# PacificBiosciences/ccs

Hardware: AMD Instinct MI355X
Metric: ZMWs/sec (HiFi reads/sec), 10-pass x 10 kb synthetic (higher is better)
Workload: dtype f32

## Files before the change

ccs_amd/csrc/ccsx_kernels.hip:

```cpp
#include <hip/hip_runtime.h>
#include <stdint.h>
#include <cstdio>
#include <cstdlib>

#include "ccsx.h"
#include "ccsx_kernels.h"
#include "wave_ops.h"

#define LANDED(x) asm volatile("" : "+v"(x))

#if (defined(CCSX_EXP_NO_FILL) || defined(CCSX_EXP_NO_SCORE) || defined(CCSX_EXP_ONE_ROUND) || defined(CCSX_EXP_ALL_VALID) || defined(CCSX_EXP_CHEAP_VALIDITY) || \
     defined(CCSX_EXP_NO_ROWS) || defined(CCSX_EXP_NO_SCORE_LOG) || defined(CCSX_EXP_SKIP_ROUND2_SCORE) || defined(CCSX_EXP_NO_QV_EXP) || defined(CCSX_EXP_REPEAT) || defined(CCSX_EXP_NO_BANDMASK) || \
     defined(CCSX_EXP_HOT_PROLOGUE) || defined(CCSX_EXIT_AFTER_PROLOGUE)) && !defined(CCSX_EXPERIMENT)
#error "CCSX_EXP_* / CCSX_EXIT_AFTER_PROLOGUE switches produce wrong results: build them with -DCCSX_EXPERIMENT (never ship such a library)"
#endif
#define CCSX_STR2(x) #x
#define CCSX_STR(x) CCSX_STR2(x)
int ccsx_kernel_is_experiment()
{
#ifdef CCSX_EXPERIMENT
    return 1;
#else
    return 0;
#endif
// ... 1656 lines not shown
                if (cf > NEGV / 2 && cf > bF) { bF = cf; kF = k; }
                if (cr > NEGV / 2 && cr > bR) { bR = cr; kR = k; }
            }
            const int wF = rfl(wave_max_i32(bF)), wR = rfl(wave_max_i32(bR));
            if (wF <= NEGV / 2 || wR <= NEGV / 2) continue;
            const int k1 = rfl(wave_min_i32(bF == wF ? kF : (1 << 30))), kr = rfl(wave_min_i32(bR == wR ? kR : (1 << 30)));
            const int k2 = nneed - 1 - kr;
            const int s1 = need_col(wb, nw, Ld, k1), s2r = Ld - need_col(wb, nw, Ld, k2);
            if (!(k1 < k2 && s1 > 0 && s2r > 0 && wF >= s1 && wR >= s2r && brF[k1] + brR[kr] <= I)) continue;
            if (lane == 0) {
                int32_t *ent = P.ent + P.ent_off[r];
                uint32_t *dm = P.dmask + P.ent_off[r];
                const int2 *OMF = (const int2 *)OsF, *OMR = (const int2 *)OsR;
                int e = ebF[k1];
                ent[k1] = e;
                for (int kq = k1; kq >= 2; --kq) { e = OMF[(size_t)kq * 64 + (e - loF[kq])].x; ent[kq - 1] = e; }
                ent[0] = 0;
                int er = ebR[kr];
                ent[k2] = I - er;
                for (int kq = kr; kq >= 1; --kq) {
                    er = (kq >= 2) ? OMR[(size_t)kq * 64 + (er - loR[kq])].x : 0;
                    ent[nneed - kq] = I - er;
                }
                for (int kq = k1 + 1; kq < k2; ++kq) ent[kq] = -(1 << 20) - 64 * kq;
                dm[0] = 0u;
                for (int kq = 1; kq < nneed; ++kq) dm[kq] = 0x7fffffffu;
                P.avalid[r] = 1; P.ascore[r] = wF + wR;
            }
            continue;
        }
        if (lane == 0) {
            int32_t *ent = P.ent + P.ent_off[r];
            uint32_t *dm = P.dmask + P.ent_off[r];
            const int2 *OMF = (const int2 *)OsF, *OMR = (const int2 *)OsR;
            int e = ks ? ebF[ks] : 0;
            ent[ks] = e;
            for (int k2 = ks; k2 >= 2; --k2) { e = OMF[(size_t)k2 * 64 + (e - loF[k2])].x; ent[k2 - 1] = e; }
            ent[0] = 0;
            const int ksr = nneed - 1 - ks;
            int er = ksr ? ebR[ksr] : 0;
            for (int kq = ksr; kq >= 1; --kq) {
                er = (kq >= 2) ? OMR[(size_t)kq * 64 + (er - loR[kq])].x : 0;
                ent[nneed - kq] = I - er;
            }
            dm[0] = 0u;
            for (int k2 = 1; k2 < nneed; ++k2) dm[k2] = 0x7fffffffu;
            P.avalid[r] = 1; P.ascore[r] = wbest;
        }
      }
    }
}

__global__ void k_post(KParams P, int pass)
{
    int z = blockIdx.x * blockDim.x + threadIdx.x;
    if (z >= P.n_zmw) return;
    const int zr = P.zref[z];
    if (pass && !(zr & ZREF_PASSBIT(pass))) return;
    const bool may_retry = !P.opts.no_fallback_draft && pass < 2;
    const int retry = pass == 0 ? ZREF_RETRY : ((zr & 255) | ZREF_RETRY2);
    if (P.zstat[z] != CCSX_SUCCESS) {
        P.np[z] = 0; P.out_fn[z] = 0; P.out_rn[z] = 0;
        if (may_retry && P.zstat[z] == CCSX_DRAFT_FAILURE) P.zref[z] = retry;
        return;
    }
    int r0 = P.read_off[z], nr = P.nfull[z], np = 0, rn = 0;
    const int f0 = P.flags[r0 + (zr & 255)];
    for (int r = 0; r < nr; ++r) {
        const int v = P.avalid[r0 + r];
        np += v;
        if (v && ((P.flags[r0 + r] ^ f0) & 1)) ++rn;
    }
    P.np[z] = np; P.out_fn[z] = np - rn; P.out_rn[z] = rn;
    if (2 * np <= nr) {
        if (may_retry) P.zref[z] = retry;
        else { P.zstat[z] = CCSX_TOO_MANY_UNUSABLE; P.nwin[z] = 0; }
    }
}

__global__ __launch_bounds__(1024) void k_wmap(KParams P)
{
    __shared__ int sTot[16], sCarry;
    const int tid = threadIdx.x, lane = tid & 63, wv = tid >> 6;
    if (tid == 0) sCarry = 0;
    __syncthreads();
    for (int z0 = 0; z0 < P.n_zmw; z0 += 1024) {
        const int z = z0 + tid;
        const int v = z < P.n_zmw ? P.nwin[z] : 0;
        const int incl = wave_scan_add_i32(v);
        if (lane == 63) sTot[wv] = incl;
        __syncthreads();
        int base = sCarry;
        for (int q = 0; q < wv; ++q) base += sTot[q];
        if (z < P.n_zmw) P.wstart[z] = base + incl - v;
        __syncthreads();
        if (tid == 1023) sCarry = base + incl;
        __syncthreads();
    }
    if (tid == 0) P.wstart[P.n_zmw] = sCarry;
}
__global__ __launch_bounds__(256) void k_wmap_fill(KParams P)
{
    const int z = blockIdx.x * 4 + (threadIdx.x >> 6), lane = threadIdx.x & 63;
    if (z >= P.n_zmw) return;
    const int a = P.wstart[z], nw = P.nwin[z];
    for (int w = lane; w < nw; w += LANES) P.wslot_zmw[a + w] = z;
}

#ifndef PW_THREADS
#define PW_THREADS 256
#endif
#ifndef PW_MINWAVES
#define PW_MINWAVES 4
#endif
#define PW_WAVES (PW_THREADS / 64)
#ifndef PW_CHUNK_READS
#define PW_CHUNK_READS 8
#endif
#ifndef PW_MAXREADS
#define PW_MAXREADS 32
#endif
#ifndef PW_LDS_BYTES
#define PW_LDS_BYTES 40960
#endif
#ifndef CTXS
#define CTXS 17
#endif
#define FILL16_MAXBW 24
#define TC_LO 56
#define TC_HI 38
#define TC_ROW 32
#define TC_STRAND ((CCSX_NOBS + 1) * TC_ROW)
#define DLC_S (33 + TC_LO)
#define DLC_TOTAL (TC_LO + DLC_S + 33 + TC_HI)
#define TAB_TAIL (2 * TC_HI - 48)
#define OBS_TC(o) ((o) * (TC_ROW * 8))
#define OBS_CODE(o) ((o) * (CTXS * 8))

struct LaneMut {
    int c, q, kA, kB, isdel, fin;
    int qoff;
    float dlA, dlL;
};

__device__ __forceinline__ LaneMut lane_mut(int type, int c, int x, const uint8_t *t, int J, int lf, const float *sDL)
{
    LaneMut L;
    const int tm1 = t[c > 0 ? c - 1 : 0];
    const int nidx = (type == 2) ? c : c + 1;
    const int tn = t[nidx < 31 ? nidx : 31];
    const int fin = (type == 2) ? (c == J) : (c + 1 == J);
    const int nx = fin ? 0 : tn;
    int pA = (c > 0) ? tm1 : lf;
    const int xA = (type == 1) ? nx : x;
    if (pA > 3) pA = (xA + 2) & 3;
    const int kA = pA * 4 + xA, kB = (type == 1) ? kA : xA * 4 + nx;
    const int q = (type == 2) ? c + 1 : c + 2;
    L.c = c; L.q = q > J ? J : q; L.isdel = (type == 1); L.fin = fin; L.qoff = (type == 2) ? 0 : 1;
    L.dlA = sDL[kA]; L.dlL = sDL[kB];
    L.kA = (type == 1 && fin) ? (CTXS - 1) : kA;
    L.kB = fin ? (CTXS - 1) : kB;
    return L;
}

typedef const float __attribute__((address_space(3))) *lds_cf;
typedef const char __attribute__((address_space(3))) *lds_cc;

typedef const uint8_t __attribute__((address_space(3))) *lds_cu8;
struct ScoreChain {
    float ap, bp, acc, b, bq;
    float2 pA, pB;
    lds_cf g, be;
    lds_cu8 op;
    int dg;
};

__device__ __forceinline__ float lanes_or_zero(unsigned long long m, float v)
{
    float r;
    asm("v_cndmask_b32_e64 %0, 0, %1, %2" : "=v"(r) : "v"(v), "s"(m));
    return r;
}

__device__ __forceinline__ void score_step(ScoreChain &s, const LaneMut &L, lds_cc tA, lds_cc tB, int pitch, unsigned lim)
{
    typedef const unsigned long long __attribute__((address_space(3))) *lds_cu64;
#ifndef CCSX_EXP_NO_BANDMASK
    const unsigned long long on = __builtin_amdgcn_uicmp((unsigned)s.dg, lim, 37 );
    const float gmm = lanes_or_zero(on, *s.g);
    const float bqn = lanes_or_zero(on, *s.be);
#else
    const float gmm = *s.g, bqn = *s.be;
#endif
    const int o256 = __mul24((int)*s.op, CTXS * 8);
    const unsigned long long va = *(lds_cu64)(tA + o256), vb = *(lds_cu64)(tB + o256);
    const float2 nA = make_float2(__uint_as_float((unsigned)va), __uint_as_float((unsigned)(va >> 32)));
    const float2 nB = make_float2(__uint_as_float((unsigned)vb), __uint_as_float((unsigned)(vb >> 32)));
    s.g += pitch; s.be += pitch; s.op += 1; s.dg -= 1;
    const float insA = s.pA.y, meA = s.pA.x, insB = s.pB.y;
    const float a = __builtin_fmaf(s.ap, insA, gmm);
    float b;
    if (L.isdel) b = a;
    else b = __builtin_fmaf(s.bp, insB, __builtin_fmaf(a, L.dlA, s.ap * meA));
    s.acc = __builtin_fmaf(b, __builtin_fmaf(L.dlL, s.bq, nB.x * bqn), s.acc);
    s.ap = a; s.bp = b; s.b = b; s.pA = nA; s.pB = nB; s.bq = bqn;
}

__device__ __forceinline__ int band_row0(int c, int I, int J2, float invJ2, int J, int Wr, int nrows)
{
    const int num = __mul24(2 * c, I) + J;
    int q = (int)((float)num * invJ2);
    const int r = num - __mul24(q, J2);
    q += (r >= J2 ? 1 : 0) - (r < 0 ? 1 : 0);
    int i0 = q - Wr;
    i0 = i0 < 0 ? 0 : i0;
    const int hi = I + 1 - nrows;
    return i0 > hi ? hi : i0;
}

__device__ __forceinline__ int dq_fix(float d)
{
    if (d < -DQ_CLAMP) d = -DQ_CLAMP;
    if (d > DQ_CLAMP) d = DQ_CLAMP;
    return (int)floorf(d * DQ_SCALE + 0.5f);
}

__device__ __forceinline__ float skip_perr(int g, float floor_)
{
    if (g < 0) g = 0;
    if (g > 12) g = 12;
    const float p = 8.0f * det_exp2f(-3.0f * (float)g);
    return p < floor_ ? floor_ : p;
}

__device__ __forceinline__ int tract_len(unsigned long long m, int x, int p, int nvis)
{
    const int lo = x - p < 0 ? 0 : x - p;
    const unsigned long long cand = m & ((2ull << x) - 1ull) & ~((1ull << lo) - 1ull);
    if (!cand) return 0;
    int best = 0;
#pragma unroll
    for (int which = 0; which < 2; ++which) {
        const int k = which ? 63 - __clzll((long long)cand) : __ffsll((long long)cand) - 1;
        const unsigned long long zb = ~m & ((1ull << k) - 1ull);
        const int i = zb ? 64 - __clzll((long long)zb) : 0;
        const int j = k + (__ffsll((long long)(~m >> k)) - 1);
        const int L = j - i + p, op = ((i == 0) || (j + p >= nvis)) ? 256 : 0;
        if (L > (best & 255)) best = L | op; else if (L == (best & 255)) best |= op;
    }
    return best;
}


struct FillBand { int dlo, dhi, bw, pitch, org, rowsz; };
__device__ __forceinline__ FillBand fill_band_of(int I, int J, int S)
{
    FillBand b;
    const int dIJ = I > J ? I - J : J - I;
    const int W = SCORE_BAND + FILL_MARGIN + (dIJ > 2 ? dIJ - 2 : 0);
    const int lo = (J - I < 0 ? J - I : 0) - W, hi = (J - I > 0 ? J - I : 0) + W;
    b.dlo = lo < -I ? -I : lo; b.dhi = hi > J ? J : hi;
    b.bw = b.dhi - b.dlo + 1;
    const int bwp = b.bw | 1;
    const bool diag = bwp < S;
    b.rowsz = diag ? bwp : S; b.pitch = diag ? bwp - 1 : S; b.org = diag ? -b.dlo : 0;
    return b;
}

__device__ __forceinline__ int polish_piece_windows(int total, int slot0, int grid) { const int c = total - slot0; return c < 0 ? 0 : (c > grid ? grid : c); }
__device__ __forceinline__ int xcd_contiguous(unsigned b, int count)
{
    const int per = (count + 7) >> 3;
    const int k = (int)(b >> 3), r = (int)(b & 7u) * per + k;
    return (k < per && r < count) ? r : -1;
}

template <int PWT, int PWMIN, int PWCH>
__global__ __launch_bounds__(PWT, PWMIN) void k_polish_t(KParams P, int slot0)
{
    __shared__ float2 sCTX[(CCSX_NOBS + 1) * CTXS];
    static_assert(DLC_TOTAL >= 2 * TC_LO && TAB_TAIL >= 0 && (DLC_TOTAL & 1) == 0, "sTab: guards / alignment of sTC");
    __shared__ __attribute__((aligned(16))) float sTab[DLC_TOTAL + 2 * TC_STRAND * 2 + 48 + TAB_TAIL];
    float *const sDLC = sTab;
    float2 *const sTC = (float2 *)(sTab + DLC_TOTAL);
    float *const sDL = sTab + DLC_TOTAL + 2 * TC_STRAND * 2, *const sZP = sDL + 16;
    __shared__ uint8_t sT[2][32];
    __shared__ uint8_t sTd[32];
    uint8_t (*sObs)[68] = (uint8_t (*)[68])dyn_lds;
    float *sGB = (float *)((uint8_t *)dyn_lds + P.pw_obs_bytes);
    const int GB_FLOATS = P.pw_gb_floats;
    __shared__ int sI[PW_MAXREADS], sGoff[PW_MAXREADS], sBoff[PW_MAXREADS];
    __shared__ int sBand[PW_MAXREADS];
    __shared__ unsigned sDirty[PW_MAXREADS];
    __shared__ uint8_t sStrand[PW_MAXREADS], sRend[PW_MAXREADS];
    __shared__ unsigned sZdrop[(CCSX_MAX_PASSES + 32) / 32];
    __shared__ float sBase[PW_MAXREADS], sB00[PW_MAXREADS];
    __shared__ short2 sTask[PW_MAXREADS];
    __shared__ int sDeltaI[256];
    float *sDelta = (float *)sDeltaI;
    __shared__ uint8_t sMvalid[256];
    __shared__ int sCtl[12];
    __shared__ float sZS[4];
    __shared__ float sPskip[36];
    __shared__ int sCnt[(PWT / 64)];
    __shared__ uint8_t sList[256];

    const int tid = threadIdx.x, lane = tid & 63, wave = rfl(tid >> 6);
    PHASE_T0();
    const int nwin_here = polish_piece_windows(P.wstart[P.n_zmw], slot0, (int)gridDim.x);
#ifdef CCSX_EXP_HOT_PROLOGUE
    const int bid_ = slot0 + xcd_contiguous(blockIdx.x, nwin_here);
    const int bid = bid_ < slot0 ? bid_ : slot0 + ((bid_ - slot0) & 4095);
#else
    const int bid = slot0 + xcd_contiguous(blockIdx.x, nwin_here);
#endif
    if (bid < slot0) return;
    const int z = P.wslot_zmw[bid];
    const int wbo = P.wb_off[z], nw = P.nwin[z], Ld = P.draft_len[z];
    const int r0 = P.read_off[z], nreads = P.nreads_used[z];
    const int64_t so = P.seq_off[z];
    const int w = bid - P.wstart[z];
    const int32_t *wb = P.wbounds + wbo;
    const uint8_t *draft = P.draft + so;
    const int wb0 = wb[w], wb1 = wb[w + 1];
    const int64_t bo_r0 = P.base_off[r0];
    const int fl0 = P.flags[r0 + (P.zref[z] & 255)] & 1;
    int ws = wb0 - CCSX_WIN_OVERHANG; if (ws < 0) ws = 0;
    int we = wb1 + CCSX_WIN_OVERHANG; if (we > Ld) we = Ld;
    const int idx_ws = (w == 0) ? 0 : 2 * w - 1, idx_we = (w == nw - 1) ? 2 * nw - 1 : 2 * (w + 1);
    const int lfv = draft[ws > 0 ? ws - 1 : 0], rfv = draft[we < Ld ? we : Ld - 1];
    const int lf = ws > 0 ? lfv : 4, rf = we < Ld ? rfv : 4;
    const int c1 = need_col(wb, nw, Ld, idx_ws + 1), c2 = (idx_ws + 2 <= idx_we) ? need_col(wb, nw, Ld, idx_ws + 2) : we;
    const int maxins = P.opts.max_insertion_size == 0 ? 30 : P.opts.max_insertion_size;
    {
        const int e0 = tid < CCSX_NOBS * 16 ? tid : 0;
        const size_t tz = (size_t)z * 192;
        const int i0 = (e0 & 15) * CCSX_NOBS + (e0 >> 4);
        const float me0 = P.tabME[tz + i0], in0 = P.tabINS[tz + i0];
        const float dl = P.tabDL[(size_t)z * 16 + (tid & 15)];
        const float zp = P.tabZ[(size_t)z * 32 + (tid & 31)];
        const int tcl = tid < we - ws ? tid : we - ws - 1;
        const uint8_t dr = draft[ws + tcl];
        if (tid < CCSX_NOBS * 16) sCTX[(e0 >> 4) * CTXS + (e0 & 15)] = make_float2(me0, in0);
        if (tid < CTXS) sCTX[CCSX_NOBS * CTXS + tid] = make_float2(0.0f, 0.0f);
        if (tid < CCSX_NOBS) sCTX[tid * CTXS + (CTXS - 1)] = make_float2(0.0f, 0.0f);
        if (tid < TAB_TAIL) sZP[32 + tid] = 0.0f;
        if (tid < 16) sDL[tid] = dl;
        if (tid < 32) sZP[tid] = zp;
        if (tid < we - ws) { sT[0][tid] = dr; sTd[tid] = dr; }
        if (tid == 0) { sCtl[0] = we - ws; sCtl[1] = wb0 - ws; sCtl[2] = wb1 - ws; }
    }
    const int ngroups = (nreads + PW_MAXREADS - 1) / PW_MAXREADS;
    auto load_meta = [&](int g0, int ng) -> int {
        int trimflag = 0;
        const int rcl = tid < ng ? tid : ng - 1;
        const int rr = r0 + g0 + rcl;
        const int64_t bo0 = P.base_off[rr], bo1 = P.base_off[rr + 1], eo = P.ent_off[rr];
        const int flr = P.flags[rr] & 1, av = P.avalid[rr];
        const int a = P.ent[eo + idx_ws], b = P.ent[eo + idx_we];
        const unsigned m1 = P.dmask[eo + idx_ws + 1];
        const unsigned m2 = (idx_ws + 2 <= idx_we) ? P.dmask[eo + idx_ws + 2] : 0u;
        const unsigned m3 = (idx_ws + 3 <= idx_we) ? P.dmask[eo + idx_ws + 3] : 0u;
        if (tid < ng) {
            const int L = (int)(bo1 - bo0);
            const int st = flr != fl0 ? 1 : 0;
            int n = -1, na = 0;
            if (av) {
                n = b - a;
                if (n > L) n = -1;
                if (n >= 0 && maxins > 0 && n > (we - ws) + maxins) { trimflag = 1; sBoff[tid] = n; n = we - ws; }
                else { sBoff[tid] = 0; if (n < 0 || n > CCSX_IMAX) n = -1; }
                na = st ? L - b : a;
            } else sBoff[tid] = 0;
            sI[tid] = n; sStrand[tid] = (uint8_t)st;
            sGoff[tid] = (int)(bo0 - bo_r0) + na;
            sDirty[tid] = av ? (m1 | (m2 << (c1 - ws)) | (m3 << (c2 - ws))) : 0u;
        }
        return trimflag;
    };
    const int glast = (ngroups > 1 ? ngroups - 1 : 0) * PW_MAXREADS;
    const int ng0 = nreads - glast < PW_MAXREADS ? nreads - glast : PW_MAXREADS;
    const int trimflag = load_meta(glast, ng0);
    int resident = glast;
    if (tid < (CCSX_MAX_PASSES + 32) / 32) sZdrop[tid] = 0u;
    auto load_obs = [&](int ng, int tflag) {
    const int anytrim = __syncthreads_or(tflag);
    for (int rb = 0; rb < ng; rb += 4 * (PWT / 64)) {
        uint8_t bq[4], pq[4];
#pragma unroll
        for (int q = 0; q < 4; ++q) {
            const int r = rb + (PWT / 64) * q + wave;
            const int n = r < ng ? sI[r] : -1;
            const int64_t p = bo_r0 + ((lane < n) ? sGoff[r] + lane : 0);
            bq[q] = P.bases[p]; pq[q] = P.pw[p];
        }
#pragma unroll
        for (int q = 0; q < 4; ++q) {
            const int r = rb + (PWT / 64) * q + wave;
            if (r < ng) {
                const int n = sI[r];
                sObs[r][lane] = (lane < n) ? (uint8_t)obs_of(bq[q], pq[q]) : (uint8_t)(lane == n ? CCSX_NOBS : 0);
                if (lane < 4) sObs[r][64 + lane] = 0;
            }
        }
    }
    if (anytrim) {
        const int J0 = we - ws;
        for (int r = wave; r < ng; r += (PWT / 64)) {
            const int nfull = rfl(sBoff[r]);
            if (nfull == 0) continue;
            const int st = rfl((int)sStrand[r]);
            const int64_t p0 = bo_r0 + sGoff[r];
            const bool in = lane < J0;
            const int bp = in ? P.bases[p0 + lane] : 0;
            const int bs = in ? P.bases[p0 + nfull - J0 + lane] : 0, ps = in ? P.pw[p0 + nfull - J0 + lane] : 0;
            const int T = in ? (st ? 3 - (int)sTd[J0 - 1 - lane] : (int)sTd[lane]) : 9;
            const unsigned long long mp = __ballot(in && (bp & 3) == T), ms = __ballot(in && (bs & 3) == T);
            const int tot = (lane <= J0) ? __popcll(mp & ((1ull << lane) - 1ull)) + __popcll(ms >> lane) : -1;
            const int sb = 63 - (rfl(wave_max_i32((tot << 6) | (63 - lane))) & 63);
            if (in && lane >= sb) sObs[r][lane] = (uint8_t)obs_of(bs, ps);
        }
    }
    };
    load_obs(ng0, trimflag);
    {
        int nuse = 0, nd = 0;
        for (int g0 = (ngroups - 1) * PW_MAXREADS; g0 >= 0; g0 -= PW_MAXREADS) {
            const int ng = nreads - g0 < PW_MAXREADS ? nreads - g0 : PW_MAXREADS;
            if (g0 != resident) {
                __syncthreads();
                const int tf = load_meta(g0, ng);
                load_obs(ng, tf);
                __syncthreads();
                resident = g0;
            }
            if (wave == 0) {
                const int vIr = lane < ng ? sI[lane] : -1;
                const unsigned vDr = lane < ng ? sDirty[lane] : 0u;
                for (int r = 0; r < ng; ++r) if (rl(vIr, r) >= 0) { ++nuse; nd += (int)(((unsigned)rl((int)vDr, r) >> (lane & 31)) & 1u); }
            }
        }
        if (wave == 0) {
            const int J0 = we - ws;
            const int margin = nuse - 2 * nd;
            const bool inw = lane < J0;
            const unsigned neg = (unsigned)__ballot(inw && margin < 0);
            const unsigned nearneg = neg | (neg << 1) | (neg << 2) | (neg << 3) | (neg >> 1) | (neg >> 2) | (neg >> 3);
            const bool noheur = P.opts.disable_heuristics || (P.tflag && (P.tflag[z] & 2));
            const bool ok = inw && !noheur && margin >= SKIP_MARGIN && !((nearneg >> lane) & 1u);
            const unsigned ev = (unsigned)__ballot(ok);
            if (lane == 0) sCtl[7] = (int)ev;
            if (lane < 36) sPskip[lane] = inw ? skip_perr(margin, P.perr_floor) : 0.0f;
        }
    }
    const int half = lane >> 5, hrow = lane & 31;
    PHASE(0);
#ifdef CCSX_EXIT_AFTER_PROLOGUE
    __syncthreads();
    if (tid == 0) P.wsum[(size_t)(P.wb_off[z] - z) + w] = (float)sI[0] + (float)sObs[0][0] + sPskip[0] + sCTX[5].x;
    return;
#endif
#ifdef CCSX_EXP_REPEAT
    __syncthreads();
    const int xr_t = sT[0][tid & 31], xr_c0 = sCtl[0], xr_c1 = sCtl[1], xr_c2 = sCtl[2], xr_c7 = sCtl[7];
    const float xr_p = sPskip[tid < 36 ? tid : 0];
    for (int xrep = 0; xrep < CCSX_EXP_REPEAT; ++xrep) {
    __syncthreads();
    if (tid < 32) sT[0][tid] = (uint8_t)xr_t;
    if (tid < 36) sPskip[tid] = xr_p;
    if (tid < (CCSX_MAX_PASSES + 32) / 32) sZdrop[tid] = 0u;
    if (tid == 0) { sCtl[0] = xr_c0; sCtl[1] = xr_c1; sCtl[2] = xr_c2; sCtl[7] = xr_c7; }
    __syncthreads();
#endif
    auto plan_chunks = [&](int ng, int J, int S) {
        int r = lane;
        asm volatile("" : "+v"(r));
        const int n0 = r < ng ? sI[r] : -1;
        const FillBand fb = fill_band_of(n0 >= 0 ? n0 : 0, J, S);
        const int need0 = (2 * n0 + 3) * fb.rowsz;
        const bool qd0 = n0 <= 31 && fb.bw <= FILL16_MAXBW;
        const unsigned long long lower = (1ull << r) - 1ull;
        for (int rb = 0; rb < ng;) {
            const bool cand = n0 >= 0 && r >= rb;
            const int need = cand ? need0 : 0;
            const int incl = wave_scan_add_i32(need);
            const unsigned long long bcand = __ballot(cand);
            const unsigned long long over = __ballot(cand && (incl > GB_FLOATS || (PWCH > 0 && __popcll(bcand & lower) >= PWCH)));
            const int rend_ = over ? (int)__ffsll((long long)over) - 1 : ng;
            if (r >= rb && r < rend_) {
                if (!cand) sGoff[r] = -1;
                else {
                    const int off = incl - need;
                    sGoff[r] = off + fb.org; sBoff[r] = off + (n0 + 1) * fb.rowsz + fb.org;
                    sBand[r] = fb.pitch | (fb.rowsz << 8) | (fb.bw << 16) | ((fb.dlo + 128) << 24);
                }
            }
            const bool inchunk = cand && r < rend_;
            const bool qd = inchunk && qd0, lng = inchunk && !qd0;
            const unsigned long long bl = __ballot(lng), bs = __ballot(qd);
            const int nl_ = __popcll(bl);
            if (lng) sTask[rb + __popcll(bl & lower)].x = (short)r;
            if (qd) sTask[rb + nl_ + __popcll(bs & lower)].x = (short)r;
            if (r == rb) { sRend[rb] = (uint8_t)rend_; sTask[rb].y = (short)(nl_ | (__popcll(bs) << 8)); }
            rb = rfl(rend_);
        }
    };
    int iters = 0, nonconv = 0;
    unsigned skmask = 0;
    int nvalid_last = 0, nvfull_last = 0;
    const int nfull = P.nfull[z];
    for (int it = 0; it < CCSX_MAX_ITER; ++it) {
        __syncthreads();
        const int J = rfl(sCtl[0]);
        const float invJ2 = 1.0f / (float)(2 * J);
        const int S = (J + 2) & ~1;
        if (tid < J) sT[1][tid] = (uint8_t)(3 - sT[0][J - 1 - tid]);
        __syncthreads();
        if (wave == (PWT / 64) - 1 && resident == 0) plan_chunks(nreads < PW_MAXREADS ? nreads : PW_MAXREADS, J, S);
        auto tbase = [&](int sd, int j) -> int { return (int)sT[sd][j]; };
        const int lfr = (rf < 4) ? 3 - rf : 4;
        if (it == 0 && wave < 2 && P.opts.min_zscore != 0.0f) {
            const int j = lane < J ? lane : 0;
            const int prev = j > 0 ? tbase(wave, j - 1) : (wave ? lfr : lf);
            const int k = ctx_of(prev, tbase(wave, j));
            const float mu = sZP[k], va = sZP[16 + k];
            float M = 0.0f, V = 0.0f;
            for (int q = 0; q < J; ++q) {
                M = M + __int_as_float(rl(__float_as_int(mu), q));
                V = V + __int_as_float(rl(__float_as_int(va), q));
            }
            if (lane == 0) { sZS[2 * wave] = M; sZS[2 * wave + 1] = V; }
        }
        {
            const uint8_t *t = sT[0];
            const int c = lane & 31;
            const int tc = c < J ? t[c] : 9;
            const int prev = c > 0 ? (c - 1 < J ? t[c - 1] : 8) : lf, next = c + 1 < J ? t[c + 1] : rf;
            const bool hp = (prev == tc) || (next == tc);
            skmask = (unsigned)__ballot(lane < J && (((unsigned)sCtl[7] >> c) & 1u) && !hp);
        }
        {
            const uint8_t *t = sT[0];
            const int sl0 = tid >> 5, c0 = tid & 31;
            int v0;
            if (sl0 < 3) v0 = c0 < J;
            else if (sl0 == 3) v0 = c0 < J && !(c0 > 0 && t[c0 - 1] == t[c0]);
            else if (sl0 < 8) v0 = c0 <= J && !(c0 > 0 && t[c0 - 1] == sl0 - 4);
            else v0 = 0;
            {
                const int cc = c0 < J ? c0 : J - 1;
                if (v0 && ((skmask >> cc) & 1u)) v0 = 0;
                else if (v0 && (((unsigned)sCtl[7] >> cc) & 1u) && !(c0 < J && (sl0 == 3 || (sl0 >= 4 && sl0 - 4 == t[c0])))) v0 = 0;
            }
            const unsigned long long bal = __ballot(v0);
            if (lane == 0) sCnt[wave] = __popcll(bal);
            if (tid < 256) { sMvalid[tid] = (uint8_t)v0; sDeltaI[tid] = 0; }
            __syncthreads();
            int basew = 0;
            for (int q = 0; q < wave; ++q) basew += sCnt[q];
            if (v0) sList[basew + __popcll(bal & ((1ull << lane) - 1ull))] = (uint8_t)tid;
            __syncthreads();
        }
        for (int e = tid; e < 2 * TC_STRAND; e += PWT) {
            const int sd = e >= TC_STRAND ? 1 : 0, e2 = e - sd * TC_STRAND, o = e2 >> 5, j = e2 & 31;
            float2 v = make_float2(0.0f, 0.0f);
            if (j < J) {
                const int prev = j > 0 ? tbase(sd, j - 1) : (sd ? lfr : lf);
                v = sCTX[o * CTXS + ctx_of(prev, tbase(sd, j))];
            }
            sTC[e] = v;
        }
        for (int e = tid; e < DLC_TOTAL; e += PWT) {
            const int sd = e >= TC_LO + 33 ? 1 : 0, j = e - TC_LO - sd * DLC_S;
            float v = 1.0f;
            if (j >= 0 && j < J) {
                const int prev = j > 0 ? tbase(sd, j - 1) : (sd ? lfr : lf);
                v = sDL[ctx_of(prev, tbase(sd, j))];
            }
            sDLC[e] = e >= DLC_TOTAL - 2 ? 0.0f : v;
        }
        int nvm = 0;
#pragma unroll
        for (int q = 0; q < (PWT / 64); ++q) nvm += rfl(sCnt[q]);
        const int nblk = (nvm + 63) >> 6;
        PHASE(1);
        int nvalid = 0, nvfull = 0;
        int curblk = -1;
        LaneMut LF, LR;
        int myM = 0; bool mval = false;
        for (int g0 = 0; g0 < nreads; g0 += PW_MAXREADS) {
        const int ng = nreads - g0 < PW_MAXREADS ? nreads - g0 : PW_MAXREADS;
        if (g0 != resident) {
            __syncthreads();
            const int tf = load_meta(g0, ng);
            load_obs(ng, tf);
            resident = g0;
            __syncthreads();
            if (wave == (PWT / 64) - 1) plan_chunks(ng, J, S);
        }
        int rbeg = 0;
        while (rbeg < ng) {
            __syncthreads();
            const int rend = rfl((int)sRend[rbeg]), ntasks = rfl((int)sTask[rbeg].y), nlong = ntasks & 255, nshort = ntasks >> 8;
            const short2 *const cTask = sTask + rbeg;
            PHASE(2);
#ifdef CCSX_EXP_NO_FILL
            const int nquad = 0, nunit_f = 0, rpq = 4;
#else
            const int rpq = 4;
            const int nquad = (nshort + rpq - 1) / rpq, nunit_f = 2 * nquad + 2 * nlong;
#endif
            for (int fu = wave; fu < nunit_f; fu += (PWT / 64)) {
              if (fu < 2 * nquad) {
                const int quad = fu >> 1, isb = fu & 1;
                const int g4 = lane >> 4, l16 = lane & 15;
                const int qi = rpq * quad + g4;
                const bool have = g4 < rpq && qi < nshort;
                const int myr = cTask[nlong + (have ? qi : rpq * quad)].x;
                const int I = sI[myr], sd = sStrand[myr], band = sBand[myr];
                const int pitch = band & 255, rowsz = (band >> 8) & 255, bdlo = (int)((unsigned)band >> 24) - 128, bdhi = bdlo + ((band >> 16) & 255) - 1;
                const int row0 = l16, row1 = l16 + 16;
                const bool ok0 = have && row0 <= I, ok1 = have && row1 <= I;
                const int jlo0 = (row0 + bdlo > 0) ? row0 + bdlo : 0, jhi0 = (row0 + bdhi < J) ? row0 + bdhi : J;
                const int jlo1 = (row1 + bdlo > 0) ? row1 + bdlo : 0, jhi1 = (row1 + bdhi < J) ? row1 + bdhi : J;
                int Tmax = 0;
#pragma unroll
                for (int q = 0; q < 4; ++q) { const int iq = rfl(sI[rfl((int)cTask[nlong + ((q < rpq && rpq * quad + q < nshort) ? rpq * quad + q : rpq * quad)].x)]); Tmax = iq > Tmax ? iq : Tmax; }
                Tmax += J;
                const int NEVER = 1 << 20;
#define LDPR(ROWP, OFF) (*(const float2 *)((ROWP) + (OFF)))
                if (!isb) {
                    const int obA0 = OBS_TC((row0 >= 1 && ok0) ? (int)sObs[myr][row0 - 1] : 12);
                    const int obA1 = OBS_TC(ok1 ? (int)sObs[myr][row1 - 1] : 12);
                    const char *tA = (const char *)(sTC + sd * TC_STRAND) + obA0 - 8 * row0;
                    const int dtA = obA1 - obA0 - 8 * 16;
                    const float *dA = sDLC + sd * DLC_S + (TC_LO - 1 - row0);
                    const int tA0 = ok0 ? row0 + jlo0 : NEVER, tA1 = row1 + jlo1;
                    unsigned uJ = ok0 ? (unsigned)(jhi0 - jlo0) : 0u;
                    const unsigned uJ1 = (unsigned)(jhi1 - jlo1);
                    const int tsw = ok1 ? ((row0 + jhi0) & ~3) : NEVER;
                    float *gA = sGB + sGoff[myr] + row0 * pitch - row0;
                    const int dgA = 16 * (pitch - 1), dcnt = tA0 - tA1;
                    float acur = (ok0 && row0 == 0) ? 1.0f : 0.0f, mnext = 0.0f;
#define CCSX_A_INIT(K) float dl##K = dA[K]; float2 p##K = LDPR(tA, 8 * (K));
                    CCSX_A_INIT(0) CCSX_A_INIT(1) CCSX_A_INIT(2) CCSX_A_INIT(3)
#undef CCSX_A_INIT
                    int cnt = -tA0;
#define CCSX_A_STEP(K)                                                                                                     \
                    {                                                                                                      \
                        const float up = row_ror1_f32(acur);                                              \
                        const float gmm = __builtin_fmaf(acur, dl##K, mnext);                         \
                        const unsigned long long on = __builtin_amdgcn_uicmp((unsigned)(cnt + (K)), uJ, 37 );    \
                        if (__builtin_amdgcn_inverse_ballot_w64(on)) gA[(K)] = gmm;                                        \
                        acur = lanes_or_zero(on, __builtin_fmaf(up, p##K.y, gmm));    \
                        mnext = up * p##K.x;                                                                               \
                        p##K = LDPR(tA, 8 * ((K) + 4));                            \
                        dl##K = dA[(K) + 4];                                                                               \
                    }
                    for (int t = 0; t <= Tmax; t += 4, tA += 32, dA += 4, gA += 4, cnt += 4) {
                        if (t == tsw) { tA += dtA; dA -= 16; }
                        if (t - 4 == tsw) { uJ = uJ1; cnt += dcnt; gA += dgA; }
                        CCSX_A_STEP(0) CCSX_A_STEP(1) CCSX_A_STEP(2) CCSX_A_STEP(3)
                    }
#undef CCSX_A_STEP
                    if (have && l16 == 0) sBase[myr] = sGB[sGoff[myr] + I * pitch + J];
                } else {
                    const int rowF = ok1 ? row1 : row0, jloF = ok1 ? jlo1 : jlo0, jhiF = ok1 ? jhi1 : jhi0;
                    const int obB0 = OBS_TC((ok0 && row0 < I) ? (int)sObs[myr][row0] : 12);
                    const int obBF = ok1 ? OBS_TC(row1 < I ? (int)sObs[myr][row1] : 12) : obB0;
                    const char *tB = (const char *)(sTC + sd * TC_STRAND) + obBF + 8 * (J + I - rowF);
                    const int dtB = obB0 - obBF + 8 * 16;
                    const float *dB = sDLC + sd * DLC_S + (TC_LO + J + I - rowF);
                    const int tB0 = ok0 ? I - rowF + J - jhiF : NEVER, tB1 = I - row0 + J - jhi0;
                    unsigned uJ = ok0 ? (unsigned)(jhiF - jloF) : 0u;
                    const unsigned uJ1 = (unsigned)(jhi0 - jlo0);
                    const int tsw = ok1 ? ((I - row1 + J - jlo1) & ~3) : NEVER;
                    float *bE = sGB + sBoff[myr] + rowF * pitch + (J + I - rowF);
                    const int dbE = -16 * (pitch - 1), dcnt = tB0 - tB1;
                    float bcur = (ok0 && rowF == I) ? 1.0f : 0.0f, t1next = 0.0f;
#define CCSX_B_INIT(K) float dk##K = dB[-(K)]; float2 q##K = LDPR(tB, -8 * (K));
                    CCSX_B_INIT(0) CCSX_B_INIT(1) CCSX_B_INIT(2) CCSX_B_INIT(3)
#undef CCSX_B_INIT
                    int cnt = -tB0;
#define CCSX_B_STEP(K, KN)                                                                                                 \
                    {                                                                                                      \
                        const float dn = row_rol1_f32(bcur);                                             \
                        const float bv = __builtin_fmaf(dk##K, bcur, __builtin_fmaf(q##K.y, dn, t1next));    \
                        const unsigned long long on = __builtin_amdgcn_uicmp((unsigned)(cnt + (K)), uJ, 37 );    \
                        if (__builtin_amdgcn_inverse_ballot_w64(on)) bE[-(K)] = bv;                                        \
                        bcur = lanes_or_zero(on, bv);                                                                      \
                        t1next = q##KN.x * dn;                        \
                        q##K = LDPR(tB, -8 * ((K) + 4));                                                                   \
                        dk##K = dB[-(K) - 4];                                                                              \
                    }
                    for (int t = 0; t <= Tmax; t += 4, tB -= 32, dB -= 4, bE -= 4, cnt += 4) {
                        if (t == tsw) { tB += dtB; dB += 16; }
                        if (t - 4 == tsw) { uJ = uJ1; cnt += dcnt; bE += dbE; }
                        CCSX_B_STEP(0, 1) CCSX_B_STEP(1, 2) CCSX_B_STEP(2, 3) CCSX_B_STEP(3, 0)
                    }
#undef CCSX_B_STEP
                    const int org_ = pitch == S ? 0 : -bdlo;
                    if (have) for (int x = l16; x < rowsz; x += 16) sGB[sBoff[myr] - org_ + (I + 1) * rowsz + x] = 0.0f;
                    if (have && l16 == 0) sB00[myr] = sGB[sBoff[myr]];
                }
#undef LDPR
              } else {
                const int tk = (fu - 2 * nquad) >> 1, mode = 1 + ((fu - 2 * nquad) & 1);
                const int myr = rfl((int)cTask[tk].x);
                const int row = lane;
                const int I = rfl(sI[myr]);
                const int Tmax = I + J;
                const int sd = sStrand[myr];
                const float *dlcol = sDLC + sd * DLC_S + TC_LO;
                const bool rowok = row <= I;
                const int band = sBand[myr];
                const int pitch = band & 255, rowsz = (band >> 8) & 255, bdlo = (int)((unsigned)band >> 24) - 128, bdhi = bdlo + ((band >> 16) & 255) - 1;
                const int jlo = (row + bdlo > 0) ? row + bdlo : 0, jhi = (row + bdhi < J) ? row + bdhi : J;
                const int op = OBS_TC((row >= 1 && rowok) ? (int)sObs[myr][row - 1] : 12);
                const int oc = OBS_TC((row < I) ? (int)sObs[myr][row] : 12);
                const float2 *rowA = (const float2 *)((const char *)(sTC + sd * TC_STRAND) + op), *rowB = (const float2 *)((const char *)(sTC + sd * TC_STRAND) + oc);
                const int tA0 = rowok ? row + jlo : (1 << 20), tB0 = rowok ? I - row + J - jhi : (1 << 20);
                const float one0 = (row == 0) ? 1.0f : 0.0f, oneI = (row == I) ? 1.0f : 0.0f;
                float *gA = sGB + sGoff[myr] + row * pitch - row;
                float *bB = sGB + sBoff[myr] + row * pitch + (J + I - row - 1);
                float acur = one0, updiag = 0.0f, mePrev = 0.0f, dlPrev = 1.0f;
                float bcur = oneI, dndiag = 0.0f;
                const unsigned uJ = rowok ? (unsigned)(jhi - jlo) : 0u;
                const int tAc = rowok ? row : (1 << 20);
                const unsigned uJc = (unsigned)J;
                if (mode == 1) {
                    for (int t = 0; t <= Tmax; t += 2, gA += 2) {
#define CCSX_LA_STEP(T, AOFF)                                                                                         \
                        {                                                                                                  \
                            const float up = wave_shr1_f32_z(acur);   \
                            float nv = 0.0f;                                                                               \
                            if ((unsigned)((T) - tAc) <= uJc) {              \
                                const float2 pr = rowA[(T) - row];                                                         \
                                const float dlc = dlcol[(T) - row];                                                        \
                                const float gmm = __builtin_fmaf(acur, dlPrev, updiag * mePrev);                           \
                                if ((unsigned)((T) - tA0) <= uJ) { gA[(AOFF)] = gmm; nv = __builtin_fmaf(up, pr.y, gmm); }    \
                                mePrev = pr.x; dlPrev = dlc;                                                               \
                            }                                                                                              \
                            acur = nv;                                                                                     \
                            updiag = up;                                                                                   \
                        }
                        CCSX_LA_STEP(t, 0)
                        CCSX_LA_STEP(t + 1, 1)
#undef CCSX_LA_STEP
                    }
                    if (lane == 0) sBase[myr] = sGB[sGoff[myr] + I * pitch + J];
                } else {
                    for (int t = 0; t <= Tmax; t += 2, bB -= 2) {
#define CCSX_LB_STEP(T, BOFF)                                                                                         \
                        {                                                                                                  \
                            const float dn = wave_shl1_f32_z(bcur);                                                        \
                            float nv = 0.0f;                                                                               \
                            if ((unsigned)((T) - tB0) <= uJ) {        \
                                const int jb = J + I - row - (T);                       \
                                const float2 pr = rowB[jb];                                                                \
                                const float bv = __builtin_fmaf(dlcol[jb], bcur, __builtin_fmaf(pr.y, dn, pr.x * dndiag)); \
                                bB[(BOFF)] = bv;                                                                           \
                                nv = bv;                                                                                   \
                            }                                                                                              \
                            bcur = nv;                                                                                     \
                            dndiag = dn;                                                                                   \
                        }
                        CCSX_LB_STEP(t, 1)
                        CCSX_LB_STEP(t + 1, 0)
#undef CCSX_LB_STEP
                    }
                    const int org_ = pitch == S ? 0 : -bdlo;
                    if (row < rowsz) sGB[sBoff[myr] - org_ + (I + 1) * rowsz + row] = 0.0f;
                    if (lane == 0) sB00[myr] = sGB[sBoff[myr]];
                }
              }
            }
            __syncthreads();
            PHASE(3);
            int vOk = 0; float vLa = 0.0f;
            if (lane >= rbeg && lane < rend && sGoff[lane] >= 0) {
                const float aIJ = sBase[lane], b00 = sB00[lane];
                const int I = sI[lane], sd = sStrand[lane];
                if (aIJ > TINY_P && b00 > TINY_P) {
#ifdef CCSX_EXP_CHEAP_VALIDITY
                    vLa = aIJ; const float lb = b00 - (b00 - aIJ);
#else
                    vLa = det_log2f(aIJ); const float lb = det_log2f(b00);
#endif
                    float df = vLa - lb; if (df < 0.0f) df = -df;
                    vOk = !(df > AB_TOL);
                    if ((sZdrop[g0 >> 5] >> lane) & 1u) vOk = 0;
                    else if (vOk && it == 0 && P.opts.min_zscore != 0.0f) {
                        const float zd = (vLa - (float)(2 * I)) - sZS[2 * sd];
                        const float zm = P.opts.min_zscore;
                        if (zd < 0.0f && zd * zd > (zm * zm) * sZS[2 * sd + 1]) { vOk = 0; atomicOr(&sZdrop[g0 >> 5], 1u << lane); }
                    }
                }
            }
#ifdef CCSX_EXP_ALL_VALID
            vOk = (lane >= rbeg && lane < rend && sGoff[lane] >= 0) ? 1 : 0;
#endif
            int vRlist, nv_chunk;
            {
                const bool v = vOk != 0;
                const unsigned long long bv = __ballot(v), lower = (1ull << lane) - 1ull;
                nv_chunk = rfl(__popcll(bv));
                nvfull += __popcll(bv & (nfull - g0 >= 64 ? ~0ull : (nfull - g0 <= 0 ? 0ull : (1ull << (nfull - g0)) - 1ull)));
                const int dest = v ? __popcll(bv & lower) : nv_chunk + __popcll(~bv & lower);
                vRlist = __builtin_amdgcn_ds_permute(dest << 2, lane);
            }
            PHASE(7);
            {
#ifdef CCSX_EXP_SKIP_ROUND2_SCORE
                const int nv = nv_chunk, nunits = (it == 0) ? nblk * nv : 0;
#elif defined(CCSX_EXP_NO_SCORE)
                const int nv = nv_chunk, nunits = 0;
#else
                const int nv = nv_chunk, nunits = nblk * nv;
#endif
                nvalid += nv;
                int vR, vI, vSt, vG, vB, vBd; float vBase;
                {
                    vR = lane < nv ? vRlist : rl(vRlist, 0);
                    vI = sI[vR]; vSt = (int)sStrand[vR]; vG = sGoff[vR]; vB = sBoff[vR]; vBd = sBand[vR]; vBase = __shfl(vLa, vR);
                }
                const int u_end = ((wave + 1) * nunits) / (PWT / 64);
                for (int u = (wave * nunits) / (PWT / 64); u < u_end;) {
                    int blk = 0, k0 = u;
                    while (k0 >= nv) { k0 -= nv; ++blk; }
                    const bool two = (u + 1 < u_end) && (k0 + 1 < nv);
                    u += two ? 2 : 1;
                    if (blk != curblk) {
                        curblk = blk;
                        const int li = blk * 64 + lane;
                        mval = li < nvm;
                        myM = mval ? sList[li] : 0;
                        const int slot = myM >> 5, cpos = myM & 31;
                        int type, x = 0;
                        const uint8_t *t = sT[0];
                        if (slot < 3) { type = 0; x = (t[cpos < J ? cpos : 0] + 1 + slot) & 3; }
                        else if (slot == 3) type = 1;
                        else { type = 2; x = slot - 4; }
                        if (mval) {
                            LF = lane_mut(type, cpos, x, sT[0], J, lf, sDL);
                            LR = lane_mut(type, (type == 2) ? J - cpos : J - 1 - cpos, 3 - x, sT[1], J, lfr, sDL);
                        } else { LF = lane_mut(0, 0, 0, sT[0], J, lf, sDL); LR = LF; }
                    }
                    int dq;
                    if (!two) {
                        const int ra = rl(vR, k0), Ia = rl(vI, k0);
                        const LaneMut La = rl(vSt, k0) ? LR : LF;
                        const int gA_ = rl(vG, k0), bA_ = rl(vB, k0), bdA = rl(vBd, k0);
                        const int pA = bdA & 255, dloA = (int)((unsigned)bdA >> 24) - 128; const unsigned bwA = (unsigned)(bdA >> 16) & 255u;
                        const int dA = Ia > J ? Ia - J : J - Ia, WrA = SCORE_BAND + (dA > 2 ? dA - 2 : 0);
#ifdef CCSX_EXP_NO_ROWS
                        const int nrA = 0;
#else
                        const int nrA = (Ia < 2 * WrA ? Ia : 2 * WrA) + 1;
#endif
                        const int i0a = band_row0(La.c, Ia, 2 * J, invJ2, J, WrA, nrA);
                        lds_cc tAa = (lds_cc)(sCTX + La.kA), tBa = (lds_cc)(sCTX + La.kB);
                        ScoreChain ca;
                        ca.ap = ca.bp = ca.acc = ca.b = 0.0f; ca.pA = ca.pB = make_float2(0.f, 0.f);
                        ca.g = (lds_cf)(sGB + gA_ + __mul24(i0a, pA) + La.c); ca.be = (lds_cf)(sGB + bA_ + __mul24(i0a, pA) + La.q);
                        ca.dg = La.c - i0a - dloA;
                        ca.bq = *ca.be; if ((unsigned)(La.q - i0a - dloA) >= bwA) ca.bq = 0.0f;
                        ca.be += pA;
                        const unsigned limA = bwA - 1u - (unsigned)La.qoff;
                        ca.op = (lds_cu8)(&sObs[ra][0] + i0a);
                        asm volatile("" : "+v"(ca.g), "+v"(ca.be), "+v"(tAa), "+v"(tBa), "+v"(ca.op));
                        {
                            int ia = 0;
                            for (; ia + 2 <= nrA; ia += 2) { score_step(ca, La, tAa, tBa, pA, limA); score_step(ca, La, tAa, tBa, pA, limA); }
                            if (ia < nrA) score_step(ca, La, tAa, tBa, pA, limA);
                        }
                        const float res = La.fin ? ca.b : ca.acc;
#ifdef CCSX_EXP_NO_SCORE_LOG
                        dq = __float_as_int(res) >> 20;
#else
                        dq = dq_fix(det_log2f(res) - __int_as_float(rl(__float_as_int(vBase), k0)));
#endif
                    } else {
                    const int k1 = k0 + 1;
                    const int ra = rl(vR, k0), rb = rl(vR, k1);
                    const int Ia = rl(vI, k0), Ib = rl(vI, k1);
                    const LaneMut La = rl(vSt, k0) ? LR : LF;
// ... 1804 lines not shown
```

Before: 39390.

## Build per-iteration template context tables with lane shuffles, dropping block barriers

Rebuilds the per-iteration setup of the polish kernel so each lane computes its template base, neighbours and reverse-complement from registers using DPP shifts and ds_bpermute instead of reading sT from LDS. The valid-mutation list is built by having every wave compute ballots for all eight slots redundantly, which removes the sCnt shared array and two __syncthreads. The sTC and sDLC context tables are filled with a fixed four-entries-per-thread mapping using the precomputed contexts. This trades duplicated ballot and validity work per wave for fewer block barriers and LDS round trips. It relies on static layout assumptions enforced by static_asserts.

```diff
diff --git a/ccs_amd/csrc/ccsx_kernels.hip b/ccs_amd/csrc/ccsx_kernels.hip
--- a/ccs_amd/csrc/ccsx_kernels.hip
+++ b/ccs_amd/csrc/ccsx_kernels.hip
@@ -1982,7 +1982,6 @@
     __shared__ int sCtl[12];
     __shared__ float sZS[4];
     __shared__ float sPskip[36];
-    __shared__ int sCnt[(PWT / 64)];
     __shared__ uint8_t sList[256];
 
     const int tid = threadIdx.x, lane = tid & 63, wave = rfl(tid >> 6);
@@ -2192,17 +2191,25 @@
     for (int it = 0; it < CCSX_MAX_ITER; ++it) {
         __syncthreads();
         const int J = rfl(sCtl[0]);
+        const unsigned evb = (unsigned)rfl(sCtl[7]);
+        int tl = tid;
+        asm volatile("" : "+v"(tl));
+        const int ll = tl & 63;
+        const int c = tl & 31;
+        const int tc = (int)sT[0][c];
         const float invJ2 = 1.0f / (float)(2 * J);
         const int S = (J + 2) & ~1;
-        if (tid < J) sT[1][tid] = (uint8_t)(3 - sT[0][J - 1 - tid]);
-        __syncthreads();
+        const int lfr = (rf < 4) ? 3 - rf : 4;
+        const int tm1 = wave_shr1_i32(tc, 0), tp1 = wave_shl1_i32(tc, 0);
+        const int rcc = 3 - __builtin_amdgcn_ds_bpermute(((J - 1 - c) & 31) << 2, tc);
+        const int rm1 = wave_shr1_i32(rcc, 0);
+        if (tl < J) sT[1][tl] = (uint8_t)rcc;
+        const int fctx = c < J ? ctx_of(c > 0 ? tm1 : lf, tc) : CTXS - 1;
+        const int rctx = c < J ? ctx_of(c > 0 ? rm1 : lfr, rcc) : CTXS - 1;
         if (wave == (PWT / 64) - 1 && resident == 0) plan_chunks(nreads < PW_MAXREADS ? nreads : PW_MAXREADS, J, S);
-        auto tbase = [&](int sd, int j) -> int { return (int)sT[sd][j]; };
-        const int lfr = (rf < 4) ? 3 - rf : 4;
         if (it == 0 && wave < 2 && P.opts.min_zscore != 0.0f) {
-            const int j = lane < J ? lane : 0;
-            const int prev = j > 0 ? tbase(wave, j - 1) : (wave ? lfr : lf);
-            const int k = ctx_of(prev, tbase(wave, j));
+            static_assert(CTXS == 17 && TAB_TAIL >= 1, "the z-score terms of a column from J on are read at sZP[CTXS - 1] and sZP[16 + CTXS - 1]");
+            const int k = wave ? rctx : fctx;
             const float mu = sZP[k], va = sZP[16 + k];
             float M = 0.0f, V = 0.0f;
             for (int q = 0; q < J; ++q) {
@@ -2212,56 +2219,55 @@
             if (lane == 0) { sZS[2 * wave] = M; sZS[2 * wave + 1] = V; }
         }
         {
-            const uint8_t *t = sT[0];
-            const int c = lane & 31;
-            const int tc = c < J ? t[c] : 9;
-            const int prev = c > 0 ? (c - 1 < J ? t[c - 1] : 8) : lf, next = c + 1 < J ? t[c + 1] : rf;
-            const bool hp = (prev == tc) || (next == tc);
-            skmask = (unsigned)__ballot(lane < J && (((unsigned)sCtl[7] >> c) & 1u) && !hp);
-        }
+            const int tcv = c < J ? tc : 9;
+            const int prev = c > 0 ? (c - 1 < J ? tm1 : 8) : lf, next = c + 1 < J ? tp1 : rf;
+            const bool hp = (prev == tcv) || (next == tcv);
+            skmask = (unsigned)__ballot(ll < J && ((evb >> c) & 1u) && !hp);
+        }
+        auto lane_valid = [&](int sl) -> int {
+            int v;
+            if (sl < 3) v = c < J;
+            else if (sl == 3) v = c < J && !(c > 0 && tm1 == tc);
+            else v = c <= J && !(c > 0 && tm1 == sl - 4);
+            const int cc = c < J ? c : J - 1;
+            if (v && ((skmask >> cc) & 1u)) v = 0;
+            else if (v && ((evb >> cc) & 1u) && !(c < J && (sl == 3 || (sl >= 4 && sl - 4 == tc)))) v = 0;
+            return v;
+        };
+        int nvm = 0;
         {
-            const uint8_t *t = sT[0];
-            const int sl0 = tid >> 5, c0 = tid & 31;
-            int v0;
-            if (sl0 < 3) v0 = c0 < J;
-            else if (sl0 == 3) v0 = c0 < J && !(c0 > 0 && t[c0 - 1] == t[c0]);
-            else if (sl0 < 8) v0 = c0 <= J && !(c0 > 0 && t[c0 - 1] == sl0 - 4);
-            else v0 = 0;
-            {
-                const int cc = c0 < J ? c0 : J - 1;
-                if (v0 && ((skmask >> cc) & 1u)) v0 = 0;
-                else if (v0 && (((unsigned)sCtl[7] >> cc) & 1u) && !(c0 < J && (sl0 == 3 || (sl0 >= 4 && sl0 - 4 == t[c0])))) v0 = 0;
-            }
-            const unsigned long long bal = __ballot(v0);
-            if (lane == 0) sCnt[wave] = __popcll(bal);
-            if (tid < 256) { sMvalid[tid] = (uint8_t)v0; sDeltaI[tid] = 0; }
-            __syncthreads();
+            static_assert(PWT == 256, "the set-up: eight slots of 32 columns, two per wave");
+            unsigned long long mine = 0ull;
             int basew = 0;
-            for (int q = 0; q < wave; ++q) basew += sCnt[q];
-            if (v0) sList[basew + __popcll(bal & ((1ull << lane) - 1ull))] = (uint8_t)tid;
-            __syncthreads();
-        }
-        for (int e = tid; e < 2 * TC_STRAND; e += PWT) {
-            const int sd = e >= TC_STRAND ? 1 : 0, e2 = e - sd * TC_STRAND, o = e2 >> 5, j = e2 & 31;
-            float2 v = make_float2(0.0f, 0.0f);
-            if (j < J) {
-                const int prev = j > 0 ? tbase(sd, j - 1) : (sd ? lfr : lf);
-                v = sCTX[o * CTXS + ctx_of(prev, tbase(sd, j))];
-            }
-            sTC[e] = v;
-        }
-        for (int e = tid; e < DLC_TOTAL; e += PWT) {
-            const int sd = e >= TC_LO + 33 ? 1 : 0, j = e - TC_LO - sd * DLC_S;
-            float v = 1.0f;
-            if (j >= 0 && j < J) {
-                const int prev = j > 0 ? tbase(sd, j - 1) : (sd ? lfr : lf);
-                v = sDL[ctx_of(prev, tbase(sd, j))];
-            }
-            sDLC[e] = e >= DLC_TOTAL - 2 ? 0.0f : v;
-        }
-        int nvm = 0;
-#pragma unroll
-        for (int q = 0; q < (PWT / 64); ++q) nvm += rfl(sCnt[q]);
+#pragma unroll
+            for (int q = 0; q < (PWT / 64); ++q) {
+                const unsigned long long b = __ballot(lane_valid(2 * q + (ll >> 5)));
+                const int n = __popcll(b);
+                if (q < wave) basew += n;
+                if (q == wave) mine = b;
+                nvm += n;
+            }
+            const int v0 = (int)((mine >> ll) & 1ull);
+            sMvalid[tl] = (uint8_t)v0; sDeltaI[tl] = 0;
+            if (v0) sList[basew + __popcll(mine & ((1ull << ll) - 1ull))] = (uint8_t)tid;
+        }
+        {
+            static_assert(PWT == 256 && TC_ROW == 32 && 2 * TC_STRAND <= 4 * PWT && DLC_TOTAL <= PWT, "the set-up: four sTC entries and one sDLC entry per thread");
+            const int row0 = tl >> 5;
+            const int ej = tl - TC_LO - (tl >= TC_LO + 33 ? DLC_S : 0);
+            const int both = __builtin_amdgcn_ds_bpermute((ej & 31) << 2, fctx | (rctx << 8));
+            float2 v[4];
+#pragma unroll
+            for (int k = 0; k < 4; ++k) {
+                const int r = row0 + 8 * k, sd = r >= CCSX_NOBS + 1 ? 1 : 0, o = r - sd * (CCSX_NOBS + 1);
+                v[k] = sCTX[r < 2 * (CCSX_NOBS + 1) ? o * CTXS + (sd ? rctx : fctx) : 0];
+            }
+            const bool inw = ej >= 0 && ej < J;
+            const float dv = sDL[inw ? (tl >= TC_LO + 33 ? both >> 8 : both & 255) : 0];
+#pragma unroll
+            for (int k = 0; k < 4; ++k) if (row0 + 8 * k < 2 * (CCSX_NOBS + 1)) sTC[tl + PWT * k] = v[k];
+            if (tl < DLC_TOTAL) sDLC[tl] = tl >= DLC_TOTAL - 2 ? 0.0f : (inw ? dv : 1.0f);
+        }
         const int nblk = (nvm + 63) >> 6;
         PHASE(1);
         int nvalid = 0, nvfull = 0;
```

Result: faster. 40360, median of 6 (+2.4%).
